# WojciechMula/pyahocorasick

Measured on NVIDIA H100. Metric: haystack GB/s, higher is better.
Workload: dtype u8

## Files before the change

### pyahocorasick_b200/csrc/acb_device.cu

```cuda
#include "acb_internal.h"
#include "acb_hash.h"

#include <cuda_runtime.h>
#include <cub/device/device_radix_sort.cuh>

#include <algorithm>
#include <atomic>
#include <mutex>
#include <chrono>
#include <cstdio>
#include <cstdlib>
#include <cstring>
#include <exception>
#include <new>
#include <vector>

#define CUDA_TRY(expr)                                                                       \
    do {                                                                                     \
        cudaError_t _e = (expr);                                                             \
        if (_e != cudaSuccess) {                                                             \
            acb_set_error("CUDA error %s at %s:%d: %s", cudaGetErrorName(_e), __FILE__,      \
                          __LINE__, cudaGetErrorString(_e));                                 \
            return ACB_ECUDA;                                                                \
        }                                                                                    \
// ... 293 lines not shown
    }
}

struct ProbeCtx {
    uint32_t sbm;
    uint32_t n_words;
    uint32_t four;
    uint32_t two;
    int sh_bit;
};

template <int N>
__device__ __forceinline__ uint32_t window(const uint32_t (&W)[N], int t) {
    return ((t & 3) == 0) ? W[t >> 2] : __funnelshift_r(W[t >> 2], W[(t >> 2) + 1], (t & 3) * 8);
}

template <int NW, int STRIDE, bool WIDE>
__device__ __forceinline__ uint32_t probe_single(const ProbeCtx &c, const uint32_t (&W)[kLaneWords + NW], const uint32_t (&mul)[NW]) {
    constexpr int kProbes = kLaneBytes / STRIDE;
    uint32_t acc = 0;
#pragma unroll
    for (int t = 0; t < kLaneBytes; t += STRIDE) {
        uint32_t h = 0, ha;
        if (WIDE) {
            unsigned long long hw = 0;
#pragma unroll
            for (int k = 0; k < NW; k++) hw = mad_wide(window(W, t + 4 * k), mul[k], hw);
            h = (uint32_t)hw;
            ha = (uint32_t)(hw >> 32);
        } else {
#pragma unroll
            for (int k = 0; k < NW; k++) h += window(W, t + 4 * k) * mul[k];
            ha = h >> c.sh_bit;
        }
        const uint32_t word = lds_bitmap(__umulhi(h, c.n_words) * c.four + c.sbm);
        const uint32_t both = __funnelshift_r(word, 0u, ha) & __funnelshift_r(word, 0u, h) & 1u;
        acc = acc * c.two + both;
    }
    return __brev(acc) >> (32 - kProbes);
}

struct StreamSmem {
    uint32_t bitmap, stages, stage_rec, stage_cnt, bars, tiles, next, total;
};
__host__ __device__ inline StreamSmem stream_smem(int log1) {
    StreamSmem s;
    uint32_t o = 0;
    s.bitmap = o;    o += 1u << (log1 - 3);                       o = (o + 127u) & ~127u;
    s.stages = o;    o += (uint32_t)kStages * kStageBytes;
    s.stage_rec = o; o += (uint32_t)kConsumers * kStageCap * (uint32_t)sizeof(acb_match);
    s.stage_cnt = o; o += (uint32_t)kConsumers * 4u;              o = (o + 15u) & ~15u;
    s.bars = o;      o += 2u * kStages * 8u;
    s.tiles = o;     o += (uint32_t)kStages * 4u;
    s.next = o;      o += 4u;
    s.total = (o + 15u) & ~15u;
    return s;
}

__device__ __forceinline__ void resolve_backlog(const ScanParams &p, uint8_t *smem_raw, unsigned int n) {
    const int lane = threadIdx.x & 31, warp = threadIdx.x >> 5;
    const StreamSmem lay = stream_smem(p.log1);
    WarpStage ws;
    ws.buf = reinterpret_cast<acb_match *>(smem_raw + lay.stage_rec) + warp * kStageCap;
    ws.cnt = reinterpret_cast<int *>(smem_raw + lay.stage_cnt) + warp;
    const uint2 *list = p.cand + ((size_t)blockIdx.x * kConsumers + warp) * kWarpCand;
    __syncwarp();
    for (unsigned int i0 = 0; i0 < n; i0 += 32) {
        const unsigned int i = i0 + lane;
        if (i < n) {
            const uint2 e = __ldcg(list + i);
            const long long q = p.seg_begin + (long long)e.x;
            uint32_t tq[6];
            load_text(p, q, tq);
            const uint32_t slot = e.y >> (32 - p.logA);
            const uint4 a0 = __ldg(p.anchors + 2 * (size_t)slot), a1 = __ldg(p.anchors + 2 * (size_t)slot + 1);
            resolve_chain(p, ws, q, e.y, tq, a0, a1);
        }
        __syncwarp();
        if (*reinterpret_cast<volatile int *>(ws.cnt) >= kStageCap / 4) flush_stage(p, ws, lane);
    }
    flush_stage(p, ws, lane);
}

template <int NCONS>
__device__ __forceinline__ void stream_producer(const ScanParams &p, uint8_t *smem_raw, uint32_t sbase, uint32_t stages,
                                                uint32_t bar_full, uint32_t bar_empty, volatile uint32_t *s_tile, int lane) {
    struct { uint32_t stages; } lay = {stages};
    const uint8_t *seg = p.hay + p.seg_begin;
    const long long exist = p.total - p.seg_begin;
    unsigned int claim[kClaimDepth];
#pragma unroll
    for (int k = 0; k < kClaimDepth; k++) claim[k] = (lane == 0) ? atomicAdd(p.work_ctr, 1u) : 0u;
    bool more = true;
    for (uint32_t base = 0; more; base += kClaimDepth) {
#pragma unroll
        for (int k = 0; k < kClaimDepth; k++) {
            if (!more) break;
            const uint32_t fill = base + k;
            const uint32_t stage = fill % kStages;
            const unsigned int tile = __shfl_sync(kFull, claim[k], 0);
            if (lane == 0 && tile < p.n_tiles) claim[k] = atomicAdd(p.work_ctr, 1u);
            if (fill >= (uint32_t)kStages) mbar_wait(bar_empty + 8u * stage, ((fill / kStages) - 1u) & 1u);
            if (tile >= p.n_tiles) {
                constexpr uint32_t kSentinels = (NCONS + kTileSlices - 1) / kTileSlices;
                static_assert(kSentinels <= (uint32_t)kStages, "sentinel fills must not wrap the ring");
                for (uint32_t k2 = 0; k2 < kSentinels; k2++) {
                    const uint32_t f2 = fill + k2, st2 = f2 % kStages;
                    if (k2 > 0 && f2 >= (uint32_t)kStages) mbar_wait(bar_empty + 8u * st2, ((f2 / kStages) - 1u) & 1u);
                    if (lane == 0) { s_tile[st2] = kNoTile; mbar_arrive(bar_full + 8u * st2); }
                }
                more = false;
                break;
            }
            const long long off = (long long)tile * kTileBytes;
            const long long avail = exist - off;
            const uint32_t want = kTileBytes + kLook;
            const uint32_t bulk = avail >= (long long)want ? want : (uint32_t)(avail & ~15LL);
            uint8_t *dst = smem_raw + lay.stages + (size_t)stage * kStageBytes;
            if (avail < (long long)want) {
                const uint32_t a = (uint32_t)avail;
                uint32_t zend = ((a + (uint32_t)kSliceBytes - 1u) & ~((uint32_t)kSliceBytes - 1u)) + kLook;
                if (zend > want) zend = want;
                for (uint32_t i = bulk + lane; i < zend; i += 32) dst[i] = i < a ? seg[off + i] : (uint8_t)0;
                __syncwarp();
            }
            if (lane == 0) {
                s_tile[stage] = tile;
                if (bulk) {
                    mbar_arrive_expect_tx(bar_full + 8u * stage, bulk);
                    bulk_load(sbase + lay.stages + stage * (uint32_t)kStageBytes, seg + off, bulk, bar_full + 8u * stage);
                } else {
                    mbar_arrive(bar_full + 8u * stage);
                }
            }
        }
    }
    {
        unsigned int sink = 0;
#pragma unroll
        for (int k = 0; k < kClaimDepth; k++) sink |= claim[k];
        if (sink == 0x7fffffffu) s_tile[0] = sink;
    }
}

template <int NW, int STRIDE, int MODE>
__global__ void __launch_bounds__(kFThreads, 1) acb_stream_kernel(const __grid_constant__ ScanParams p) {
    extern __shared__ __align__(128) uint8_t smem_raw[];
    const StreamSmem lay = stream_smem(p.log1);
    const uint32_t sbase = (uint32_t)__cvta_generic_to_shared(smem_raw);
    const int tid = threadIdx.x, lane = tid & 31, warp = tid >> 5;
    const uint32_t bar_full = sbase + lay.bars, bar_empty = bar_full + 8u * kStages;
    volatile uint32_t *s_tile = reinterpret_cast<volatile uint32_t *>(smem_raw + lay.tiles);

    {
        const int n16 = 1 << (p.log1 - 7);
        const uint4 *src = reinterpret_cast<const uint4 *>(p.bm1);
        for (int i = tid; i < n16; i += kFThreads)
            asm volatile("cp.async.cg.shared.global [%0], [%1], 16;" :: "r"(sbase + lay.bitmap + 16u * i), "l"(src + i));
        asm volatile("cp.async.commit_group;");
        if (tid < kConsumers) reinterpret_cast<int *>(smem_raw + lay.stage_cnt)[tid] = 0;
        if (tid == 0) *reinterpret_cast<unsigned int *>(smem_raw + lay.next) = 0u;
        if (tid == 0) {
            for (int s = 0; s < kStages; s++) {
                mbar_init(bar_full + 8u * s, 1);
                mbar_init(bar_empty + 8u * s, kTileSlices);
            }
            asm volatile("fence.mbarrier_init.release.cluster;" ::: "memory");
        }
        asm volatile("cp.async.wait_group 0;" ::: "memory");
    }
    __syncthreads();

    const uint32_t seg_len = (uint32_t)(p.seg_end - p.seg_begin);

    if (warp == kConsumers) {
        stream_producer<kConsumers>(p, smem_raw, sbase, lay.stages, bar_full, bar_empty, s_tile, lane);
    } else {
        ProbeCtx c;
        c.sbm = sbase + lay.bitmap;
        c.n_words = 1u << (p.log1 - 5);
        c.four = 4u + (uint32_t)(p.log1 >> 8);
        c.two = 2u + (uint32_t)(p.log1 >> 8);
        c.sh_bit = 32 - p.log1;
        const uint32_t lt_mask = (1u << lane) - 1u;
        uint32_t mul[NW];
#pragma unroll
        for (int k = 0; k < NW; k++) mul[k] = p.mul1[k];
        uint2 *list = p.cand + ((size_t)blockIdx.x * kConsumers + warp) * kWarpCand;
        uint32_t mul2[NW];
#pragma unroll
        for (int k = 0; k < NW; k++) mul2[k] = p.mul2[k];
        volatile uint16_t *items = reinterpret_cast<volatile uint16_t *>(smem_raw + lay.stage_rec + (size_t)warp * kStageCap * sizeof(acb_match));
        constexpr int kItemCap = kStageCap * (int)sizeof(acb_match) / 2;
        constexpr int kPendBits = kLaneBytes / STRIDE;
        unsigned int *s_next = reinterpret_cast<unsigned int *>(smem_raw + lay.next);
        unsigned int n_cand = 0;

        for (;;) {
            unsigned int g = 0;
            if (lane == 0) g = atomicAdd(s_next, 1u);
            g = __shfl_sync(kFull, g, 0);
            const uint32_t fill = g / (uint32_t)kTileSlices, slice_off = (g % (uint32_t)kTileSlices) * (uint32_t)kSliceBytes;
            const uint32_t stage = fill % (uint32_t)kStages;
            mbar_wait(bar_full + 8u * stage, (fill / (uint32_t)kStages) & 1u);
            const uint32_t tile = s_tile[stage];
            if (tile == kNoTile) break;
            const uint32_t tile_off = tile * (uint32_t)kTileBytes;
            const uint32_t n_valid = (seg_len - tile_off < (uint32_t)kTileBytes) ? seg_len - tile_off : (uint32_t)kTileBytes;
            if (slice_off < n_valid) {
                const uint32_t slice_saddr = sbase + lay.stages + stage * (uint32_t)kStageBytes + slice_off;
                const uint32_t saddr = slice_saddr + (uint32_t)lane * kLaneBytes;
                uint32_t W[kLaneWords + NW];
#pragma unroll
                for (int i = 0; i < kLaneWords; i += 4) {
                    const uint4 v = lds128(saddr + 4u * i);
                    W[i] = v.x; W[i + 1] = v.y; W[i + 2] = v.z; W[i + 3] = v.w;
                }
#pragma unroll
                for (int k = 0; k < NW; k++) W[kLaneWords + k] = __shfl_down_sync(kFull, W[k], 1);
                if (lane == 31) {
#pragma unroll
                    for (int k = 0; k < NW; k++) W[kLaneWords + k] = lds32(saddr + kLaneBytes + 4u * k);
                }
                uint32_t pend;
#ifdef ACB_EXP_NOPROBE
                pend = (W[0] ^ W[3] ^ W[kLaneWords]) == 0x12345678u ? 1u : 0u;
#else
                pend = probe_single<NW, STRIDE, MODE == kModeWide>(c, W, mul);
#endif
                if (n_valid - slice_off < (uint32_t)kSliceBytes) {
                    const int v = (int)(n_valid - slice_off) - lane * kLaneBytes;
                    const int valid = (v + STRIDE - 1) / STRIDE;
                    pend = (valid <= 0) ? 0u : ((valid >= 32) ? pend : (pend & ((1u << valid) - 1u)));
                }
#ifdef ACB_EXP_NOSURV
                if (pend == 0x9e3779b9u) s_tile[0] = 1u;
                pend = 0;
#endif
                if (__ballot_sync(kFull, pend != 0)) {
                    const unsigned int total = __reduce_add_sync(kFull, (unsigned int)__popc(pend));
                    const int nparts = (total > (unsigned int)kItemCap && kPendBits > 8) ? kPendBits / 8 : 1;
                    for (int part = 0; part < nparts; part++) {
                        uint32_t m = nparts > 1 ? ((pend >> (8 * part)) & 0xffu) : pend;
                        const int cnt = __popc(m);
                        int incl = cnt;
#pragma unroll
                        for (int d = 1; d < 32; d <<= 1) {
                            const int v = __shfl_up_sync(kFull, incl, d);
                            if (lane >= d) incl += v;
                        }
                        const int tot = __shfl_sync(kFull, incl, 31);
                        int at = incl - cnt;
                        while (m) {
                            const int bit = __ffs(m) - 1;
                            m &= m - 1;
                            items[at++] = (uint16_t)((lane << 5) | (bit + (nparts > 1 ? 8 * part : 0)));
                        }
                        __syncwarp();
                        for (int base = 0; base < tot; base += 32) {
                            bool ok0 = false;
                            uint32_t pos0 = 0, tag0 = 0;
                            if (base + lane < tot) {
                                const uint32_t it = items[base + lane];
                                const uint32_t t = (it >> 5) * (uint32_t)kLaneBytes + (it & 31u) * (uint32_t)STRIDE;
                                const uint32_t ga = slice_saddr + t, wa = ga & ~3u, sh = (ga & 3u) * 8u;
                                pos0 = tile_off + slice_off + t;
                                {
                                    uint32_t w0 = lds32(wa);
#pragma unroll
                                    for (int k = 0; k < NW; k++) {
                                        const uint32_t w1 = lds32(wa + 4u * (k + 1));
                                        tag0 += __funnelshift_r(w0, w1, sh) * mul2[k];
                                        w0 = w1;
                                    }
                                    tag0 |= 1u;
                                    ok0 = true;
                                }
                            }
                            if (p.log3) {
                                const uint32_t i0 = (tag0 * ACB_TAGMAP_MIX) >> (32 - p.log3);
                                if (ok0) ok0 = ((__ldg(p.bm3 + (i0 >> 5)) >> (i0 & 31u)) & 1u) != 0u;
                            }
#ifndef ACB_EXP_NODRAIN
                            const unsigned m0 = __ballot_sync(kFull, ok0);
                            if (ok0) list[n_cand + __popc(m0 & lt_mask)] = make_uint2(pos0, tag0);
                            n_cand += __popc(m0);
#else
                            if (ok0 && tag0 == pos0) s_tile[0] = 2u;
#endif
                        }
                        __syncwarp();
                    }
                }
            }
            __syncwarp();
            if (lane == 0) mbar_arrive(bar_empty + 8u * stage);
            if (n_cand >= 32u) { resolve_backlog(p, smem_raw, n_cand); n_cand = 0; }
        }
        if (n_cand) resolve_backlog(p, smem_raw, n_cand);
    }
    __syncthreads();
    if (tid == 0) {
        __threadfence();
        unsigned int done = atomicAdd(p.work_ctr + 1, 1u);
        if (done == gridDim.x - 1) {
            p.work_ctr[0] = 0u;
            p.work_ctr[1] = 0u;
            __threadfence();
        }
    }
}

#ifndef ACB_PAIR_CONSUMERS
#define ACB_PAIR_CONSUMERS 27
#endif
constexpr int kPairConsumers = ACB_PAIR_CONSUMERS;
constexpr int kPairThreads = (kPairConsumers + 1) * 32;
static_assert((kPairConsumers + kTileSlices - 1) / kTileSlices + 2 < 2 * ACB_STAGES && kPairThreads <= 1024, "pair kernel shape");
constexpr int kPairRing = 64;
constexpr int kPairItems = 64;

struct PairSmem {
    uint32_t bitmap, bitmap2, stages, ring, items, bars, tiles, next, total;
};
__host__ __device__ inline PairSmem pair_smem(int log1, int log2b) {
    PairSmem s;
    uint32_t o = 0;
    s.bitmap = o;    o += 1u << (log1 - 3);
    s.bitmap2 = o;   o += 1u << (log2b - 3);                      o = (o + 127u) & ~127u;
    s.stages = o;    o += (uint32_t)kStages * kStageBytes;
    s.ring = o;      o += (uint32_t)kPairConsumers * kPairRing * 8u;
    s.items = o;     o += (uint32_t)kPairConsumers * kPairItems * 2u;
    s.bars = o;      o += 2u * kStages * 8u;
    s.tiles = o;     o += (uint32_t)kStages * 4u;
    s.next = o;      o += 4u;
    s.total = (o + 15u) & ~15u;
    return s;
}

__device__ __forceinline__ void emit_direct(const ScanParams &p, int32_t h, int32_t e, int32_t k) {
    const unsigned long long g = atomicAdd(p.count, 1ULL);
    if (g < (unsigned long long)p.cap) { acb_match m; m.hay_id = h; m.end_index = e; m.key_id = k; p.out[g] = m; }
}

__device__ __noinline__ void pair_resolve_general(const ScanParams &p, long long q, uint32_t tag, uint32_t slot, uint4 e0, uint4 e1) {
    const uint32_t amask = (1u << p.logA) - 1u;
    long long h = -1, hs = 0, he = 0;
    for (;;) {
        if (e0.x == 0u) break;
        if (e0.x == tag) {
            const uint32_t kw[5] = {e0.w, e1.x, e1.y, e1.z, e1.w};
            const int j = (int)(e0.z & 0xffu), len = (int)((e0.z >> 8) & 0xffu);
            const int32_t kid = (int32_t)e0.y;
            if (h < 0) find_haystack(p, q, h, hs, he);
            const long long start = q - j;
            if (start >= hs && start + len <= he) {
                uint32_t ts[6];
                load_text(p, start, ts);
                if (text_equals(ts, start, len, kw)) {
                    if (kid >= 0) {
                        emit_direct(p, (int32_t)h, (int32_t)(((start + len - hs) >> p.letter_shift) - 1), kid);
                    } else {
                        int32_t st = 0;
                        for (long long i = start; i < he; ++i) {
                            const int c = __ldg(p.cls + p.hay[i]);
                            const int32_t nx = __ldg(p.gto + (long long)c * p.S + st);
                            if (nx < 0) break;
                            st = nx & kIdMask;
                            if (nx & kTermBit) emit_direct(p, (int32_t)h, (int32_t)((i - hs + 1) / p.L - 1), __ldg(p.key_of + st));
                        }
                    }
                }
            }
            if (e0.z & 0x10000u) break;
        }
        slot = (slot + 1) & amask;
        e0 = __ldg(p.anchors + 2 * (size_t)slot);
        e1 = __ldg(p.anchors + 2 * (size_t)slot + 1);
    }
}

__device__ __noinline__ void pair_resolve(const ScanParams &p, uint32_t sring, unsigned int head, unsigned int n) {
    const int lane = threadIdx.x & 31;
    const uint32_t lt_mask = (1u << lane) - 1u;
    bool hit = false;
    int32_t rh = 0, re = 0, rk = 0;
    if ((unsigned)lane < n) {
        const uint32_t amask = (1u << p.logA) - 1u;
        const uint2 e = lds64(sring + (((head + (unsigned)lane) & (kPairRing - 1u)) << 3));
        const long long q = p.seg_begin + (long long)e.x;
        uint32_t tq[6];
        load_text(p, q, tq);
        uint32_t slot = e.y >> (32 - p.logA);
        uint4 e0 = __ldg(p.anchors + 2 * (size_t)slot), e1 = __ldg(p.anchors + 2 * (size_t)slot + 1);
        while (e0.x != 0u && e0.x != e.y) {
            slot = (slot + 1) & amask;
            e0 = __ldg(p.anchors + 2 * (size_t)slot);
            e1 = __ldg(p.anchors + 2 * (size_t)slot + 1);
        }
        if (e0.x != 0u) {
            if ((int32_t)e0.y >= 0 && (e0.z & 0x100ffu) == 0x10000u) {
                const uint32_t kw[5] = {e0.w, e1.x, e1.y, e1.z, e1.w};
                const int len = (int)((e0.z >> 8) & 0xffu);
                long long h, hs, he;
                find_haystack(p, q, h, hs, he);
                hit = q + len <= he && text_equals(tq, q, len, kw);
                rh = (int32_t)h;
                re = (int32_t)(((q + len - hs) >> p.letter_shift) - 1);
                rk = (int32_t)e0.y;
            } else {
                pair_resolve_general(p, q, e.y, slot, e0, e1);
            }
        }
    }
    const unsigned mh = __ballot_sync(kFull, hit);
    if (mh) {
        unsigned long long base = 0;
        if (lane == 0) base = atomicAdd(p.count, (unsigned long long)__popc(mh));
        base = __shfl_sync(kFull, base, 0) + (unsigned long long)__popc(mh & lt_mask);
        if (hit && base < (unsigned long long)p.cap) { acb_match m; m.hay_id = rh; m.end_index = re; m.key_id = rk; p.out[base] = m; }
    }
}

__device__ __forceinline__ uint32_t probe_pair_run(uint32_t acc, uint32_t sbm, uint32_t n_words, uint32_t four, const uint32_t (&R)[5], uint32_t mulp) {
#pragma unroll
    for (int x = 0; x < 16; x += 2) {
#ifdef ACB_EXP_L1_NOWIDE
        const uint32_t hc = window(R, x + 1) * mulp, hb = hc >> 7;
#else
        const unsigned long long pr = mul_wide(window(R, x + 1), mulp);
        const uint32_t hc = (uint32_t)pr, hb = (uint32_t)(pr >> 32);
#endif
#ifdef ACB_EXP_L1_SHIFTIDX
        const uint32_t waddr = (hc >> 17) * four + sbm;
#else
        const uint32_t waddr = __umulhi(hc, n_words) * four + sbm;
#endif
#ifdef ACB_EXP_L1_NOLDS
        const uint32_t word = waddr;
#else
        const uint32_t word = lds_bitmap(waddr);
#endif
        const uint32_t ta = __funnelshift_l(0u, word, window(R, x));
        const uint32_t tb = __funnelshift_l(0u, word, hb);
#ifdef ACB_L1_CARRY
        asm("{ .reg .u32 t2; add.cc.u32 t2, %1, %1; addc.u32 %0, %0, %0; add.cc.u32 t2, %2, %2; addc.u32 %0, %0, %0; }"
            : "+r"(acc) : "r"(ta), "r"(tb));
#else
        acc = __funnelshift_l(ta, acc, 1);
        acc = __funnelshift_l(tb, acc, 1);
#endif
    }
    return acc;
}

template <int L2B>
__global__ void __launch_bounds__(kPairThreads, 1) acb_pair_kernel(const __grid_constant__ ScanParams p) {
    extern __shared__ __align__(128) uint8_t smem_raw[];
    const PairSmem lay = pair_smem(p.log1, p.log2b);
    const uint32_t sbase = (uint32_t)__cvta_generic_to_shared(smem_raw);
    const int tid = threadIdx.x, lane = tid & 31, warp = tid >> 5;
    const uint32_t bar_full = sbase + lay.bars, bar_empty = bar_full + 8u * kStages;
    volatile uint32_t *s_tile = reinterpret_cast<volatile uint32_t *>(smem_raw + lay.tiles);

    if (tid == 0) {
        *reinterpret_cast<unsigned int *>(smem_raw + lay.next) = 0u;
        for (int s = 0; s < kStages; s++) {
            mbar_init(bar_full + 8u * s, 1);
            mbar_init(bar_empty + 8u * s, kTileSlices);
        }
        asm volatile("fence.mbarrier_init.release.cluster;" ::: "memory");
    }
    __syncthreads();

    const uint32_t seg_len = (uint32_t)(p.seg_end - p.seg_begin);

    if (warp == kPairConsumers) {
        stream_producer<kPairConsumers>(p, smem_raw, sbase, lay.stages, bar_full, bar_empty, s_tile, lane);
    } else {
        {
            const int n16 = (1 << (p.log1 - 7)) + (1 << (p.log2b - 7));
            const uint4 *src = reinterpret_cast<const uint4 *>(p.bm1);
            for (int i = tid; i < n16; i += kPairConsumers * 32)
                asm volatile("cp.async.cg.shared.global [%0], [%1], 16;" :: "r"(sbase + lay.bitmap + 16u * i), "l"(src + i));
            asm volatile("cp.async.commit_group;");
            asm volatile("cp.async.wait_group 0;" ::: "memory");
            asm volatile("bar.sync 1, %0;" :: "n"(kPairConsumers * 32) : "memory");
        }
        const uint32_t sbm = sbase + lay.bitmap, sbm2 = sbase + lay.bitmap2;
        const uint32_t n_words = 1u << (p.log1 - 5);
        const int l2b = L2B ? L2B : p.log2b;
        const int shy_w = 37 - l2b, shy_a = 32 - l2b, shy_b = 27 - l2b;
        const uint32_t four = 4u + (uint32_t)(p.log1 >> 8);
        const uint32_t mulp = acb_pair_mul() + (uint32_t)(p.log1 >> 8);
        const uint32_t mul2 = p.mul2[0];
        const uint32_t lt_mask = (1u << lane) - 1u;
        const uint32_t sring = sbase + lay.ring + (uint32_t)warp * (kPairRing * 8u);
        const uint32_t sitems = sbase + lay.items + (uint32_t)warp * (kPairItems * 2u);
        const uint32_t snext = sbase + lay.next;
        const uint32_t lane5 = (uint32_t)lane << 5;
        unsigned int n_cand = 0, head = 0;

        for (;;) {
            unsigned int g = 0;
            if (lane == 0) asm volatile("atom.shared.add.u32 %0, [%1], 1;" : "=r"(g) : "r"(snext) : "memory");
            g = __shfl_sync(kFull, g, 0);
            const uint32_t fill = g / (uint32_t)kTileSlices, slice_off = (g % (uint32_t)kTileSlices) * (uint32_t)kSliceBytes;
            const uint32_t stage = fill % (uint32_t)kStages;
            mbar_wait(bar_full + 8u * stage, (fill / (uint32_t)kStages) & 1u);
            const uint32_t tile = s_tile[stage];
            if (tile == kNoTile) break;
            const uint32_t tile_off = tile * (uint32_t)kTileBytes;
            const uint32_t n_valid = (seg_len - tile_off < (uint32_t)kTileBytes) ? seg_len - tile_off : (uint32_t)kTileBytes;
            const uint32_t slice_saddr = sbase + lay.stages + stage * (uint32_t)kStageBytes + slice_off;
            const uint32_t pos_base = tile_off + slice_off;
            uint32_t pend = 0;
            if (slice_off < n_valid) {
                const uint32_t saddr = slice_saddr + (uint32_t)lane * 16u;
                uint32_t R0[5], R1[5];
                {
                    const uint4 v = lds128(saddr), u = lds128(saddr + 512u);
                    R0[0] = v.x; R0[1] = v.y; R0[2] = v.z; R0[3] = v.w;
                    R1[0] = u.x; R1[1] = u.y; R1[2] = u.z; R1[3] = u.w;
                }
                R0[4] = __shfl_down_sync(kFull, R0[0], 1);
                R1[4] = __shfl_down_sync(kFull, R1[0], 1);
                const uint32_t r1_first = __shfl_sync(kFull, R1[0], 0);
                if (lane == 31) { R0[4] = r1_first; R1[4] = lds32(slice_saddr + (uint32_t)kSliceBytes); }
#ifdef ACB_EXP_NOPROBE
                pend = (R0[0] ^ R0[3] ^ R0[4] ^ R1[1] ^ R1[4]) == 0x12345678u ? 1u : 0u;
#else
                pend = probe_pair_run(0u, sbm, n_words, four, R0, mulp);
                pend = probe_pair_run(pend, sbm, n_words, four, R1, mulp);
                pend = __brev(pend);
#endif
                if (n_valid - slice_off < (uint32_t)kSliceBytes) {
                    const int v0 = (int)(n_valid - slice_off) - lane * 16, v1 = v0 - 512;
                    const uint32_t m0 = v0 <= 0 ? 0u : (v0 >= 16 ? 0xffffu : ((1u << v0) - 1u));
                    const uint32_t m1 = v1 <= 0 ? 0u : (v1 >= 16 ? 0xffffu : ((1u << v1) - 1u));
                    pend &= m0 | (m1 << 16);
                }
#ifdef ACB_EXP_NOSURV
                if (pend == 0x9e3779b9u) s_tile[0] = 1u;
                pend = 0;
#endif
            }
            unsigned int tot = __reduce_add_sync(kFull, (unsigned)__popc(pend));
            while (tot) {
                unsigned int n_items;
                if (tot <= (unsigned)kPairItems) {
                    const unsigned int cnt = (unsigned)__popc(pend);
                    unsigned int incl = cnt;
#pragma unroll
                    for (int d = 1; d < 32; d <<= 1) {
                        const unsigned int v = __shfl_up_sync(kFull, incl, d);
                        if (lane >= d) incl += v;
                    }
                    uint32_t at = sitems + 2u * (incl - cnt);
                    while (pend) {
                        const uint32_t z = (uint32_t)__clz((int)pend);
                        pend ^= 0x80000000u >> z;
                        sts16(at, lane5 | (z ^ 31u));
                        at += 2u;
                    }
                    n_items = tot;
                    tot = 0;
                } else {
                    n_items = 0;
                    do {
                        const unsigned int mp = __ballot_sync(kFull, pend != 0u);
                        if (pend) {
                            const uint32_t z = (uint32_t)__clz((int)pend);
                            pend ^= 0x80000000u >> z;
                            sts16(sitems + 2u * (n_items + (unsigned)__popc(mp & lt_mask)), lane5 | (z ^ 31u));
                        }
                        n_items += (unsigned)__popc(mp);
                    } while (n_items <= (unsigned)(kPairItems - 32));
                    tot -= n_items;
                }
                __syncwarp();
                for (unsigned int base = 0; base < n_items;) {
                    if (n_cand == (unsigned)kPairRing) {
                        __syncwarp();
                        pair_resolve(p, sring, head, 32u); head += 32u; n_cand -= 32u;
                        continue;
                    }
                    unsigned int take = n_items - base;
                    if (take > 32u) take = 32u;
                    if (take > (unsigned)kPairRing - n_cand) take = (unsigned)kPairRing - n_cand;
                    bool ok = false;
                    uint32_t pos = 0, tag = 0;
                    if ((unsigned)lane < take) {
                        const uint32_t it = lds16(sitems + 2u * (base + (unsigned)lane));
                        const uint32_t y = it & 31u;
                        const uint32_t t = ((it >> 1) & 0x1f0u) + ((y & 16u) * 31u + y);
                        const uint32_t ga = slice_saddr + t, wa = ga & ~3u;
                        const uint32_t lo = lds32(wa), hi = lds32(wa + 4u);
                        const uint32_t w = __funnelshift_r(lo, hi, ga << 3);
                        tag = (w * mul2) | 1u;
                        const uint32_t word = lds_bitmap((tag >> shy_w) * four + sbm2);
                        ok = (__funnelshift_r(word, 0u, tag >> shy_a) & __funnelshift_r(word, 0u, tag >> shy_b) & 1u) != 0u;
                        pos = pos_base + t;
                    }
                    if (p.log3) {
                        const uint32_t i0 = (tag * ACB_TAGMAP_MIX) >> (32 - p.log3);
                        if (ok) ok = ((__ldg(p.bm3 + (i0 >> 5)) >> (i0 & 31u)) & 1u) != 0u;
                    }
#ifdef ACB_EXP_NODRAIN
                    if (ok && tag == pos) s_tile[0] = 2u;
#else
                    const unsigned mk = __ballot_sync(kFull, ok);
                    if (ok) {
                        const uint32_t at = sring + (((head + n_cand + (unsigned)__popc(mk & lt_mask)) & (kPairRing - 1u)) << 3);
                        asm volatile("st.shared.v2.u32 [%0], {%1, %2};" :: "r"(at), "r"(pos), "r"(tag) : "memory");
                    }
                    n_cand += (unsigned)__popc(mk);
#endif
                    base += take;
                }
                __syncwarp();
            }
            __syncwarp();
            if (lane == 0) mbar_arrive(bar_empty + 8u * stage);
            while (n_cand >= 32u) { pair_resolve(p, sring, head, 32u); head += 32u; n_cand -= 32u; }
        }
        if (n_cand) { __syncwarp(); pair_resolve(p, sring, head, n_cand); }
    }
    __syncthreads();
    if (tid == 0) {
        __threadfence();
        unsigned int done = atomicAdd(p.work_ctr + 1, 1u);
        if (done == gridDim.x - 1) {
            p.work_ctr[0] = 0u;
            p.work_ctr[1] = 0u;
            __threadfence();
        }
    }
}


__global__ void __launch_bounds__(kDfaThreads) acb_dfa_kernel(const ScanParams p) {
    const long long span = (long long)blockIdx.x * blockDim.x + threadIdx.x;
    const long long a = span * kDfaSpan;
    if (a >= p.total) return;
    const long long b = (a + kDfaSpan < p.total) ? a + kDfaSpan : p.total;
    long long h, hs, he;
    find_haystack(p, a, h, hs, he);
    long long i = a - p.max_key_bytes;
    if (i < hs) i = hs;
    int32_t st = 0;
    const int L = p.L;
    for (; i < b; ++i) {
        while (i >= he) {
            h += 1; hs = he;
            he = (p.offsets == nullptr) ? hs + p.stride_bytes : __ldg(p.offsets + h + 1);
            st = 0;
        }
        const long long col = (long long)__ldg(p.cls + p.hay[i]) * p.S;
        int32_t nx;
        while ((nx = __ldg(p.gto + col + st)) < 0 && st != 0) st = __ldg(p.fail + st);
        st = (nx < 0) ? 0 : (nx & kIdMask);
        if (i >= a && st != 0 && ((i + 1 - hs) % L) == 0) {
            const int32_t o0 = __ldg(p.out_ptr + st), o1 = __ldg(p.out_ptr + st + 1);
            for (int32_t o = o0; o < o1; ++o) {
                const int32_t k = __ldg(p.out_idx + o);
                const long long kb = (long long)__ldg(p.key_len + k) * L;
                if (i + 1 - kb < hs) continue;
                unsigned long long g = atomicAdd(p.count, 1ULL);
                if (g < (unsigned long long)p.cap) {
                    acb_match m;
                    m.hay_id = (int32_t)h;
                    m.end_index = (int32_t)((i - hs + 1) / L - 1);
                    m.key_id = k;
                    p.out[g] = m;
                }
            }
        }
    }
}

__device__ __forceinline__ int32_t letter_step(const ScanParams &p, int32_t st, const uint8_t *letter) {
    for (int b = 0; b < p.L; b++) {
        const int32_t nx = __ldg(p.gto + (long long)__ldg(p.cls + letter[b]) * p.S + st);
        if (nx < 0) return -1;
        st = nx & kIdMask;
    }
    return st;
}

__global__ void __launch_bounds__(kDfaThreads) acb_long_kernel(const __grid_constant__ ScanParams p) {
    const long long h = (long long)blockIdx.x * blockDim.x + threadIdx.x;
    if (h >= p.n_hay) return;
    const long long hs = p.offsets ? __ldg(p.offsets + h) : h * p.stride_bytes;
    const long long he = p.offsets ? __ldg(p.offsets + h + 1) : hs + p.stride_bytes;
    const long long n = (he - hs) / p.L;
    const uint8_t *text = p.hay + hs;
    int32_t state = (h == 0) ? p.long_init : 0, last_node = -1;
    long long index = -1, last_index = -1;
    for (;;) {
        if (last_node >= 0) {
            unsigned long long g = atomicAdd(p.count, 1ULL);
            if (g < (unsigned long long)p.cap) {
                acb_match m;
// ... 176 lines not shown


constexpr int kMaxDevices = 64;

template <int NW, int STRIDE, int MODE>
static int launch_stream_m(const ScanParams &p, int grid, cudaStream_t s) {
    auto kern = acb_stream_kernel<NW, STRIDE, MODE>;
    const size_t smem = stream_smem(p.log1).total;
    static std::atomic<size_t> opted_dev[kMaxDevices];
    int dev = 0;
    CUDA_TRY(cudaGetDevice(&dev));
    std::atomic<size_t> &opted = opted_dev[dev % kMaxDevices];
    if (opted.load(std::memory_order_relaxed) < smem) {
        CUDA_TRY(cudaFuncSetAttribute(kern, cudaFuncAttributeMaxDynamicSharedMemorySize, (int)smem));
        opted.store(smem, std::memory_order_relaxed);
    }
    kern<<<grid, kFThreads, smem, s>>>(p);
    CUDA_TRY(cudaGetLastError());
    g_launches.fetch_add(1);
    return ACB_OK;
}

static int launch_pair(const ScanParams &p, int grid, cudaStream_t s) {
    const size_t smem = pair_smem(p.log1, p.log2b).total;
    static std::atomic<size_t> opted_dev[kMaxDevices];
    int dev = 0;
    CUDA_TRY(cudaGetDevice(&dev));
    std::atomic<size_t> &opted = opted_dev[dev % kMaxDevices];
    if (opted.load(std::memory_order_relaxed) < smem) {
        CUDA_TRY(cudaFuncSetAttribute(acb_pair_kernel<17>, cudaFuncAttributeMaxDynamicSharedMemorySize, (int)smem));
        CUDA_TRY(cudaFuncSetAttribute(acb_pair_kernel<0>, cudaFuncAttributeMaxDynamicSharedMemorySize, (int)smem));
        opted.store(smem, std::memory_order_relaxed);
    }
    if (p.log2b == 17) acb_pair_kernel<17><<<grid, kPairThreads, smem, s>>>(p);
    else acb_pair_kernel<0><<<grid, kPairThreads, smem, s>>>(p);
    CUDA_TRY(cudaGetLastError());
    g_launches.fetch_add(1);
    return ACB_OK;
}

template <int NW, int STRIDE>
static int launch_stream_t(const ScanParams &p, int flags, int grid, cudaStream_t s) {
    if (flags & ACB_FILTER_PAIR) {
        if (NW != 1 || STRIDE != 1 || p.gram != 4 || p.L != 1 || p.log2b < 13 || p.log2b > 19) { acb_set_error("PAIR filter needs gram 4, stride 1, 1-byte letters and a level 2"); return ACB_EINVAL; }
        return launch_pair(p, grid, s);
    }
    if (flags & ACB_FILTER_WIDE) {
        if (p.gram != 4 * NW) { acb_set_error("WIDE filter with gram %d", p.gram); return ACB_EINVAL; }
        return launch_stream_m<NW, STRIDE, kModeWide>(p, grid, s);
    }
    return launch_stream_m<NW, STRIDE, kModeNarrow>(p, grid, s);
}

template <int NW>
static int launch_stream_s(const ScanParams &p, int flags, int stride, int grid, cudaStream_t s) {
    switch (stride) {
        case 1:  return launch_stream_t<NW, 1>(p, flags, grid, s);
        case 2:  return launch_stream_t<NW, 2>(p, flags, grid, s);
        case 4:  return launch_stream_t<NW, 4>(p, flags, grid, s);
        case 8:  return launch_stream_t<NW, 8>(p, flags, grid, s);
        case 16: return launch_stream_t<NW, 16>(p, flags, grid, s);
    }
    acb_set_error("unsupported filter stride %d", stride);
    return ACB_EINVAL;
}

static int launch_stream(const ScanParams &p, int flags, int stride, int grid, cudaStream_t s) {
    switch ((p.gram + 3) / 4) {
        case 1: return launch_stream_s<1>(p, flags, stride, grid, s);
        case 2: return launch_stream_s<2>(p, flags, stride, grid, s);
        case 3: return launch_stream_s<3>(p, flags, stride, grid, s);
        case 4: return launch_stream_s<4>(p, flags, stride, grid, s);
    }
    acb_set_error("unsupported gram length %d", p.gram);
    return ACB_EINVAL;
}

static int launch_filter_range(acb_table *tb, ScanParams &p, long long begin, long long end, cudaStream_t s) {
    if (!(tb->filter_flags & ACB_FILTER_PAIR) && !tb->d_cand) {
        CUDA_TRY(cudaMalloc(reinterpret_cast<void **>(&tb->d_cand), (size_t)tb->sm_count * kConsumers * kWarpCand * sizeof(uint2)));
        tb->dev_bytes += (long long)tb->sm_count * kConsumers * kWarpCand * (long long)sizeof(uint2);
    }
    p.cand = tb->d_cand;
    for (long long seg = begin; seg < end; seg += kSegBytes) {
        p.seg_begin = seg;
        p.seg_end = std::min<long long>(seg + kSegBytes, end);
        p.n_tiles = (unsigned int)((p.seg_end - p.seg_begin + kTileBytes - 1) / kTileBytes);
        const int grid = (int)std::min<long long>(tb->sm_count, p.n_tiles);
        int rc = launch_stream(p, tb->filter_flags, tb->stride, grid, s);
        if (rc != ACB_OK) return rc;
    }
    return ACB_OK;
}

static void fill_params(const acb_table *tb, ScanParams &p, const uint8_t *d_hay, int64_t total_bytes, const int64_t *d_offsets,
                        int64_t n_hay, int64_t stride_bytes, acb_match *d_out, int64_t cap, int64_t *d_count) {
    memset(&p, 0, sizeof(p));
    p.hay = d_hay; p.total = total_bytes; p.offsets = reinterpret_cast<const long long *>(d_offsets);
    p.n_hay = n_hay; p.stride_bytes = stride_bytes;
    p.cls = tb->d_cls; p.gto = tb->d_goto; p.fail = tb->d_fail; p.letter_fail = tb->d_lfail; p.key_of = tb->d_keyof;
    p.out_ptr = tb->d_outptr; p.out_idx = tb->d_outidx; p.key_len = tb->d_keylen;
    p.S = tb->S; p.L = tb->L; p.gram = tb->gram; p.max_key_bytes = tb->max_key_bytes;
    p.bm1 = tb->d_bm1; p.bm3 = tb->d_bm3; p.anchors = reinterpret_cast<const uint4 *>(tb->d_anchors);
    p.log1 = tb->log1; p.log3 = tb->log3; p.logA = tb->logA; p.log2b = tb->log2b;
    memcpy(p.mul1, tb->mul1, sizeof(p.mul1));
    memcpy(p.mul2, tb->mul2, sizeof(p.mul2));
    p.out = d_out; p.cap = cap; p.count = reinterpret_cast<unsigned long long *>(d_count);
    p.work_ctr = tb->d_work;
    p.stride_shift = -1;
    if (!d_offsets) for (int b = 0; b < 62; b++) if ((1LL << b) == stride_bytes) p.stride_shift = b;
    p.letter_shift = tb->L == 4 ? 2 : (tb->L == 2 ? 1 : 0);
}

static void long_scan_without_launch(acb_table *tb) {
    tb->long_final_host = tb->long_init;
    tb->long_init = 0;
}

extern "C" int acb_scan_device(acb_table *tb, const uint8_t *d_hay, int64_t total_bytes,
                               const int64_t *d_offsets, int64_t n_hay, int64_t stride_bytes,
                               acb_match *d_out, int64_t cap, int64_t *d_count, void *stream, int algo) {
    if (!tb || !d_count || total_bytes < 0 || n_hay < 0 || cap < 0 || (cap > 0 && !d_out)) { acb_set_error("bad argument"); return ACB_EINVAL; }
    if (n_hay > 0x7fffffffLL) { acb_set_error("more than 2^31-1 haystacks in one batch"); return ACB_ERANGE; }
    if (!d_offsets) {
        if (stride_bytes <= 0 || stride_bytes % tb->L || stride_bytes * n_hay != total_bytes) {
            acb_set_error("fixed-stride batch needs stride_bytes > 0, a multiple of letter_bytes, and n_hay*stride == total_bytes");
            return ACB_EINVAL;
        }
        if (stride_bytes / tb->L > 0x7fffffffLL) { acb_set_error("haystack longer than 2^31-1 letters"); return ACB_ERANGE; }
    }
    if (total_bytes == 0 || n_hay == 0) {
        if (algo == ACB_ALGO_LONG) long_scan_without_launch(tb);
        return ACB_OK;
    }
    if (reinterpret_cast<uintptr_t>(d_hay) & 15) { acb_set_error("d_hay must be 16-byte aligned"); return ACB_EINVAL; }
    CUDA_TRY(cudaSetDevice(tb->device));
    cudaStream_t s = reinterpret_cast<cudaStream_t>(stream);

    ScanParams p;
    fill_params(tb, p, d_hay, total_bytes, d_offsets, n_hay, stride_bytes, d_out, cap, d_count);

    if (algo == ACB_ALGO_AUTO) algo = ACB_ALGO_FILTER;
    if (tb->n_keys == 0) {
        if (algo == ACB_ALGO_LONG) long_scan_without_launch(tb);
        return ACB_OK;
    }
    const bool timing = g_timing.load() != 0;
    if (timing) {
        if (!tb->ev0) { CUDA_TRY(cudaEventCreate(&tb->ev0)); CUDA_TRY(cudaEventCreate(&tb->ev1)); }
        CUDA_TRY(cudaEventRecord(tb->ev0, s));
    }
    if (algo == ACB_ALGO_FILTER) {
        int rc = launch_filter_range(tb, p, 0, total_bytes, s);
        if (rc != ACB_OK) return rc;
    } else if (algo == ACB_ALGO_DFA) {
        long long spans = (total_bytes + kDfaSpan - 1) / kDfaSpan;
        long long grid = (spans + kDfaThreads - 1) / kDfaThreads;
        if (grid > 0x7fffffffLL) { acb_set_error("batch too large for one launch"); return ACB_ERANGE; }
        acb_dfa_kernel<<<(unsigned)grid, kDfaThreads, 0, s>>>(p);
        cudaError_t e = cudaGetLastError();
        if (e != cudaSuccess) { acb_set_error("DFA kernel launch failed: %s", cudaGetErrorString(e)); return ACB_ECUDA; }
        g_launches.fetch_add(1);
    } else if (algo == ACB_ALGO_LONG) {
        if (!tb->d_long_final) CUDA_TRY(cudaMalloc(reinterpret_cast<void **>(&tb->d_long_final), sizeof(int32_t)));
        p.long_init = tb->long_init;
        p.long_final = tb->d_long_final;
        tb->long_init = 0;
        tb->long_final_host = -1;
        long long grid = (n_hay + kDfaThreads - 1) / kDfaThreads;
        acb_long_kernel<<<(unsigned)grid, kDfaThreads, 0, s>>>(p);
// ... 337 lines not shown
```

Measured before the change: 1279.

## Give pair kernel its own tile/stage shape and fast path for small candidate slices

Parameterises the stream producer by tile slices and stage count, so the pair-filter kernel can use its own power-of-two tile size (32 slices) and stage count (2), computed with shifts and masks. It adds a single-round fast path when a slice yields at most 32 pending items, skipping the general item loop and ring-capacity checks. Lane 0 is now chosen with elect.sync for the shared-counter atomic, and item offsets are stored directly instead of re-decoding a packed form. This changes shared-memory footprint and pipeline depth for the pair kernel, which may affect occupancy and how well loads overlap with compute.

```diff
diff --git a/pyahocorasick_b200/csrc/acb_device.cu b/pyahocorasick_b200/csrc/acb_device.cu
--- a/pyahocorasick_b200/csrc/acb_device.cu
+++ b/pyahocorasick_b200/csrc/acb_device.cu
@@ -399,9 +399,12 @@
     flush_stage(p, ws, lane);
 }
 
-template <int NCONS>
+template <int NCONS, int TSLICES, int STAGES>
 __device__ __forceinline__ void stream_producer(const ScanParams &p, uint8_t *smem_raw, uint32_t sbase, uint32_t stages,
                                                 uint32_t bar_full, uint32_t bar_empty, volatile uint32_t *s_tile, int lane) {
+    constexpr int kTileSlices = TSLICES, kStages = STAGES;
+    constexpr int kTileBytes = kTileSlices * kSliceBytes;
+    constexpr int kStageBytes = (kTileBytes + kLook + 127) / 128 * 128;
     struct { uint32_t stages; } lay = {stages};
     const uint8_t *seg = p.hay + p.seg_begin;
     const long long exist = p.total - p.seg_begin;
@@ -491,7 +494,7 @@
     const uint32_t seg_len = (uint32_t)(p.seg_end - p.seg_begin);
 
     if (warp == kConsumers) {
-        stream_producer<kConsumers>(p, smem_raw, sbase, lay.stages, bar_full, bar_empty, s_tile, lane);
+        stream_producer<kConsumers, kTileSlices, kStages>(p, smem_raw, sbase, lay.stages, bar_full, bar_empty, s_tile, lane);
     } else {
         ProbeCtx c;
         c.sbm = sbase + lay.bitmap;
@@ -633,9 +636,24 @@
 #endif
 constexpr int kPairConsumers = ACB_PAIR_CONSUMERS;
 constexpr int kPairThreads = (kPairConsumers + 1) * 32;
-static_assert((kPairConsumers + kTileSlices - 1) / kTileSlices + 2 < 2 * ACB_STAGES && kPairThreads <= 1024, "pair kernel shape");
+#ifndef ACB_PAIR_TILE_SLICES
+#define ACB_PAIR_TILE_SLICES 32
+#endif
+#ifndef ACB_PAIR_STAGES
+#define ACB_PAIR_STAGES 2
+#endif
+constexpr int kPairTileSlices = ACB_PAIR_TILE_SLICES;
+constexpr int kPairStages     = ACB_PAIR_STAGES;
+constexpr int kPairTileLog    = __builtin_ctz(kPairTileSlices);
+constexpr int kPairStageLog   = __builtin_ctz(kPairStages);
+constexpr int kPairTileBytes  = kPairTileSlices * kSliceBytes;
+constexpr int kPairStageBytes = (kPairTileBytes + kLook + 127) / 128 * 128;
+static_assert((kPairTileSlices & (kPairTileSlices - 1)) == 0 && (kPairStages & (kPairStages - 1)) == 0 && kSliceBytes == 1024,
+              "pair ring: power-of-two tiles and stages of 1 KiB slices");
+static_assert((kPairConsumers + kPairTileSlices - 1) / kPairTileSlices + 2 < 2 * kPairStages && kPairThreads <= 1024, "pair kernel shape");
 constexpr int kPairRing = 64;
 constexpr int kPairItems = 64;
+static_assert(kPairRing >= 31 + 32, "a one-round slice must fit the ring next to a turn not yet resolved");
 
 struct PairSmem {
     uint32_t bitmap, bitmap2, stages, ring, items, bars, tiles, next, total;
@@ -645,11 +663,11 @@
     uint32_t o = 0;
     s.bitmap = o;    o += 1u << (log1 - 3);
     s.bitmap2 = o;   o += 1u << (log2b - 3);                      o = (o + 127u) & ~127u;
-    s.stages = o;    o += (uint32_t)kStages * kStageBytes;
+    s.stages = o;    o += (uint32_t)kPairStages * kPairStageBytes;
     s.ring = o;      o += (uint32_t)kPairConsumers * kPairRing * 8u;
     s.items = o;     o += (uint32_t)kPairConsumers * kPairItems * 2u;
-    s.bars = o;      o += 2u * kStages * 8u;
-    s.tiles = o;     o += (uint32_t)kStages * 4u;
+    s.bars = o;      o += 2u * kPairStages * 8u;
+    s.tiles = o;     o += (uint32_t)kPairStages * 4u;
     s.next = o;      o += 4u;
     s.total = (o + 15u) & ~15u;
     return s;
@@ -777,14 +795,14 @@
     const PairSmem lay = pair_smem(p.log1, p.log2b);
     const uint32_t sbase = (uint32_t)__cvta_generic_to_shared(smem_raw);
     const int tid = threadIdx.x, lane = tid & 31, warp = tid >> 5;
-    const uint32_t bar_full = sbase + lay.bars, bar_empty = bar_full + 8u * kStages;
+    const uint32_t bar_full = sbase + lay.bars, bar_empty = bar_full + 8u * kPairStages;
     volatile uint32_t *s_tile = reinterpret_cast<volatile uint32_t *>(smem_raw + lay.tiles);
 
     if (tid == 0) {
         *reinterpret_cast<unsigned int *>(smem_raw + lay.next) = 0u;
-        for (int s = 0; s < kStages; s++) {
+        for (int s = 0; s < kPairStages; s++) {
             mbar_init(bar_full + 8u * s, 1);
-            mbar_init(bar_empty + 8u * s, kTileSlices);
+            mbar_init(bar_empty + 8u * s, kPairTileSlices);
         }
         asm volatile("fence.mbarrier_init.release.cluster;" ::: "memory");
     }
@@ -793,7 +811,7 @@
     const uint32_t seg_len = (uint32_t)(p.seg_end - p.seg_begin);
 
     if (warp == kPairConsumers) {
-        stream_producer<kPairConsumers>(p, smem_raw, sbase, lay.stages, bar_full, bar_empty, s_tile, lane);
+        stream_producer<kPairConsumers, kPairTileSlices, kPairStages>(p, smem_raw, sbase, lay.stages, bar_full, bar_empty, s_tile, lane);
     } else {
         {
             const int n16 = (1 << (p.log1 - 7)) + (1 << (p.log2b - 7));
@@ -815,25 +833,73 @@
         const uint32_t sring = sbase + lay.ring + (uint32_t)warp * (kPairRing * 8u);
         const uint32_t sitems = sbase + lay.items + (uint32_t)warp * (kPairItems * 2u);
         const uint32_t snext = sbase + lay.next;
-        const uint32_t lane5 = (uint32_t)lane << 5;
+        const uint32_t sstages = sbase + lay.stages;
+        const uint32_t lane16 = (uint32_t)lane << 4;
         unsigned int n_cand = 0, head = 0;
+
+        auto offset_of = [&](uint32_t y) { return lane16 + y + (y & 16u) * 31u; };
+        auto top_bit = [](uint32_t m) { uint32_t y; asm("bfind.u32 %0, %1;" : "=r"(y) : "r"(m)); return y; };
+        auto list_all = [&](uint32_t pend) {
+            const unsigned int cnt = (unsigned)__popc(pend);
+            unsigned int incl = cnt;
+#pragma unroll
+            for (int d = 1; d < 32; d <<= 1) {
+                const unsigned int v = __shfl_up_sync(kFull, incl, d);
+                if (lane >= d) incl += v;
+            }
+            uint32_t at = sitems + 2u * (incl - cnt);
+            while (pend) {
+                const uint32_t y = top_bit(pend);
+                pend ^= 1u << y;
+                sts16(at, offset_of(y));
+                at += 2u;
+            }
+        };
+        auto item_round = [&](uint32_t slice_saddr, uint32_t pos_base, unsigned int base, unsigned int take) {
+            uint32_t ok = 0, pos = 0, tag = 0;
+            if ((unsigned)lane < take) {
+                const uint32_t t = lds16(sitems + 2u * (base + (unsigned)lane));
+                const uint32_t ga = slice_saddr + t, wa = ga & ~3u;
+                const uint32_t lo = lds32(wa), hi = lds32(wa + 4u);
+                const uint32_t w = __funnelshift_r(lo, hi, ga << 3);
+                tag = (w * mul2) | 1u;
+                const uint32_t word = lds_bitmap((tag >> shy_w) * four + sbm2);
+                ok = __funnelshift_r(word, 0u, tag >> shy_a) & __funnelshift_r(word, 0u, tag >> shy_b) & 1u;
+                pos = pos_base + t;
+            }
+            if (p.log3) {
+                const uint32_t i0 = (tag * ACB_TAGMAP_MIX) >> (32 - p.log3);
+                if (ok) ok = (__ldg(p.bm3 + (i0 >> 5)) >> (i0 & 31u)) & 1u;
+            }
+#ifdef ACB_EXP_NODRAIN
+            if (ok && tag == pos) s_tile[0] = 2u;
+#else
+            const unsigned mk = __ballot_sync(kFull, ok);
+            if (ok) {
+                const uint32_t at = sring + (((head + n_cand + (unsigned)__popc(mk & lt_mask)) & (kPairRing - 1u)) << 3);
+                asm volatile("st.shared.v2.u32 [%0], {%1, %2};" :: "r"(at), "r"(pos), "r"(tag) : "memory");
+            }
+            n_cand += (unsigned)__popc(mk);
+#endif
+        };
 
         for (;;) {
             unsigned int g = 0;
-            if (lane == 0) asm volatile("atom.shared.add.u32 %0, [%1], 1;" : "=r"(g) : "r"(snext) : "memory");
+            asm volatile("{ .reg .pred e; elect.sync _|e, 0xffffffff; @e atom.shared.add.u32 %0, [%1], 1; }"
+                         : "+r"(g) : "r"(snext) : "memory");
             g = __shfl_sync(kFull, g, 0);
-            const uint32_t fill = g / (uint32_t)kTileSlices, slice_off = (g % (uint32_t)kTileSlices) * (uint32_t)kSliceBytes;
-            const uint32_t stage = fill % (uint32_t)kStages;
-            mbar_wait(bar_full + 8u * stage, (fill / (uint32_t)kStages) & 1u);
+            const uint32_t fill = g >> kPairTileLog, stage = fill & (kPairStages - 1u);
+            const uint32_t slice_off = (g & (kPairTileSlices - 1u)) * (uint32_t)kSliceBytes;
+            mbar_wait(bar_full + 8u * stage, (fill >> kPairStageLog) & 1u);
             const uint32_t tile = s_tile[stage];
             if (tile == kNoTile) break;
-            const uint32_t tile_off = tile * (uint32_t)kTileBytes;
-            const uint32_t n_valid = (seg_len - tile_off < (uint32_t)kTileBytes) ? seg_len - tile_off : (uint32_t)kTileBytes;
-            const uint32_t slice_saddr = sbase + lay.stages + stage * (uint32_t)kStageBytes + slice_off;
+            const uint32_t tile_off = tile * (uint32_t)kPairTileBytes;
+            const uint32_t n_valid = (seg_len - tile_off < (uint32_t)kPairTileBytes) ? seg_len - tile_off : (uint32_t)kPairTileBytes;
+            const uint32_t slice_saddr = sstages + stage * (uint32_t)kPairStageBytes + slice_off;
             const uint32_t pos_base = tile_off + slice_off;
             uint32_t pend = 0;
             if (slice_off < n_valid) {
-                const uint32_t saddr = slice_saddr + (uint32_t)lane * 16u;
+                const uint32_t saddr = slice_saddr + lane16;
                 uint32_t R0[5], R1[5];
                 {
                     const uint4 v = lds128(saddr), u = lds128(saddr + 512u);
@@ -863,79 +929,47 @@
 #endif
             }
             unsigned int tot = __reduce_add_sync(kFull, (unsigned)__popc(pend));
-            while (tot) {
-                unsigned int n_items;
-                if (tot <= (unsigned)kPairItems) {
-                    const unsigned int cnt = (unsigned)__popc(pend);
-                    unsigned int incl = cnt;
-#pragma unroll
-                    for (int d = 1; d < 32; d <<= 1) {
-                        const unsigned int v = __shfl_up_sync(kFull, incl, d);
-                        if (lane >= d) incl += v;
+            if (tot <= 32u) {
+                if (tot) {
+                    list_all(pend);
+                    __syncwarp();
+                    item_round(slice_saddr, pos_base, 0u, tot);
+                }
+            } else {
+                while (tot) {
+                    unsigned int n_items;
+                    if (tot <= (unsigned)kPairItems) {
+                        list_all(pend);
+                        n_items = tot;
+                        tot = 0;
+                    } else {
+                        n_items = 0;
+                        do {
+                            const unsigned int mp = __ballot_sync(kFull, pend != 0u);
+                            if (pend) {
+                                const uint32_t y = top_bit(pend);
+                                pend ^= 1u << y;
+                                sts16(sitems + 2u * (n_items + (unsigned)__popc(mp & lt_mask)), offset_of(y));
+                            }
+                            n_items += (unsigned)__popc(mp);
+                        } while (n_items <= (unsigned)(kPairItems - 32));
+                        tot -= n_items;
                     }
-                    uint32_t at = sitems + 2u * (incl - cnt);
-                    while (pend) {
-                        const uint32_t z = (uint32_t)__clz((int)pend);
-                        pend ^= 0x80000000u >> z;
-                        sts16(at, lane5 | (z ^ 31u));
-                        at += 2u;
+                    __syncwarp();
+                    for (unsigned int base = 0; base < n_items;) {
+                        if (n_cand == (unsigned)kPairRing) {
+                            __syncwarp();
+                            pair_resolve(p, sring, head, 32u); head += 32u; n_cand -= 32u;
+                            continue;
+                        }
+                        unsigned int take = n_items - base;
+                        if (take > 32u) take = 32u;
+                        if (take > (unsigned)kPairRing - n_cand) take = (unsigned)kPairRing - n_cand;
+                        item_round(slice_saddr, pos_base, base, take);
+                        base += take;
                     }
-                    n_items = tot;
-                    tot = 0;
-                } else {
-                    n_items = 0;
-                    do {
-                        const unsigned int mp = __ballot_sync(kFull, pend != 0u);
-                        if (pend) {
-                            const uint32_t z = (uint32_t)__clz((int)pend);
-                            pend ^= 0x80000000u >> z;
-                            sts16(sitems + 2u * (n_items + (unsigned)__popc(mp & lt_mask)), lane5 | (z ^ 31u));
-                        }
-                        n_items += (unsigned)__popc(mp);
-                    } while (n_items <= (unsigned)(kPairItems - 32));
-                    tot -= n_items;
+                    __syncwarp();
                 }
-                __syncwarp();
-                for (unsigned int base = 0; base < n_items;) {
-                    if (n_cand == (unsigned)kPairRing) {
-                        __syncwarp();
-                        pair_resolve(p, sring, head, 32u); head += 32u; n_cand -= 32u;
-                        continue;
-                    }
-                    unsigned int take = n_items - base;
-                    if (take > 32u) take = 32u;
-                    if (take > (unsigned)kPairRing - n_cand) take = (unsigned)kPairRing - n_cand;
-                    bool ok = false;
-                    uint32_t pos = 0, tag = 0;
-                    if ((unsigned)lane < take) {
-                        const uint32_t it = lds16(sitems + 2u * (base + (unsigned)lane));
-                        const uint32_t y = it & 31u;
-                        const uint32_t t = ((it >> 1) & 0x1f0u) + ((y & 16u) * 31u + y);
-                        const uint32_t ga = slice_saddr + t, wa = ga & ~3u;
-                        const uint32_t lo = lds32(wa), hi = lds32(wa + 4u);
-                        const uint32_t w = __funnelshift_r(lo, hi, ga << 3);
-                        tag = (w * mul2) | 1u;
-                        const uint32_t word = lds_bitmap((tag >> shy_w) * four + sbm2);
-                        ok = (__funnelshift_r(word, 0u, tag >> shy_a) & __funnelshift_r(word, 0u, tag >> shy_b) & 1u) != 0u;
-                        pos = pos_base + t;
-                    }
-                    if (p.log3) {
-                        const uint32_t i0 = (tag * ACB_TAGMAP_MIX) >> (32 - p.log3);
-                        if (ok) ok = ((__ldg(p.bm3 + (i0 >> 5)) >> (i0 & 31u)) & 1u) != 0u;
-                    }
-#ifdef ACB_EXP_NODRAIN
-                    if (ok && tag == pos) s_tile[0] = 2u;
-#else
-                    const unsigned mk = __ballot_sync(kFull, ok);
-                    if (ok) {
-                        const uint32_t at = sring + (((head + n_cand + (unsigned)__popc(mk & lt_mask)) & (kPairRing - 1u)) << 3);
-                        asm volatile("st.shared.v2.u32 [%0], {%1, %2};" :: "r"(at), "r"(pos), "r"(tag) : "memory");
-                    }
-                    n_cand += (unsigned)__popc(mk);
-#endif
-                    base += take;
-                }
-                __syncwarp();
             }
             __syncwarp();
             if (lane == 0) mbar_arrive(bar_empty + 8u * stage);
@@ -1278,10 +1312,11 @@
         tb->dev_bytes += (long long)tb->sm_count * kConsumers * kWarpCand * (long long)sizeof(uint2);
     }
     p.cand = tb->d_cand;
+    const long long tile_bytes = (tb->filter_flags & ACB_FILTER_PAIR) ? kPairTileBytes : kTileBytes;
     for (long long seg = begin; seg < end; seg += kSegBytes) {
         p.seg_begin = seg;
         p.seg_end = std::min<long long>(seg + kSegBytes, end);
-        p.n_tiles = (unsigned int)((p.seg_end - p.seg_begin + kTileBytes - 1) / kTileBytes);
+        p.n_tiles = (unsigned int)((p.seg_end - p.seg_begin + tile_bytes - 1) / tile_bytes);
         const int grid = (int)std::min<long long>(tb->sm_count, p.n_tiles);
         int rc = launch_stream(p, tb->filter_flags, tb->stride, grid, s);
         if (rc != ACB_OK) return rc;
```

New measurement: 1447, median of 6. 1.13x the previous value.
